# maxsonate/video-diffusion-nnx

Measured on AMD Instinct MI355X. Metric: denoised frames/sec, 16fx64x64 1000-step DDPM, higher is better.
Workload: dtype bf16; 1 GPU; config_v2_2 (north-star shape): Unet3D dim=64 C=1, 16f x 64x64, DDPM T=1000 p_sample_loop (UNet forward + p_sample per step, hipGraph replay); value = n_gpus*B*F/(T*s_per_step); batch_per_gpu=64, parallelism=dp1 (independent samples, no collective), mfma_operands=bf16, storage=weights fp32 master, activations bf16, fp32 accumulate, process_group=none (single process)

## Files before the change

### video_diffusion_nnx_amd/csrc/conv_pw.hip

```cpp
#include "vdx_common.h"
#include "vdx_internal.h"

namespace vdx {

typedef unsigned pu32x4 __attribute__((ext_vector_type(4)));

template <int ROWS, int KS = 4, bool OUT32 = false>
__global__ __launch_bounds__(512) void conv1x1_pw_kernel(const ConvArgs P, const int nct, const int groups_per_range, const int ngroups) {
    using M = Mma<MODE_BF16>;
    constexpr int TM = ROWS / 16, TN = 2;
    constexpr int KBB = KS * 64;
    extern __shared__ __attribute__((aligned(16))) char smem[];
    const int Cin = P.C0 + P.C1, nkb = Cin / (32 * KS);
    const int WRS = Cin * 2 + 16;
    char* Wl = smem;
    float* bl = reinterpret_cast<float*>(Wl + ROWS * WRS);

    const int tid = threadIdx.x, lane = tid & 63, wave = tid >> 6, lp = lane & 15, q = lane >> 4;
    const int ct = (blockIdx.x >> 3) % nct, range = ((blockIdx.x >> 3) / nct) * 8 + (blockIdx.x & 7);
    const int co0 = ct * ROWS;
    const int g0 = range * groups_per_range, g1 = min(g0 + groups_per_range, ngroups);
    if (g0 >= g1) return;

    {
        const int cpr = Cin >> 3;
        const char* wsrc = reinterpret_cast<const char*>(P.wp);
        for (int i = tid; i < ROWS * cpr; i += 512) {
            const int row = i / cpr, c = i - row * cpr;
            const int tm = row >> 4, rr = row & 15;
            const int co = co0 + (tm >> 1) * 32 + (rr >> 2) * 8 + (tm & 1) * 4 + (rr & 3);
            *reinterpret_cast<uint4*>(Wl + row * WRS + c * 16) = *reinterpret_cast<const uint4*>(wsrc + ((size_t)(P.wrow0 + co) * P.CinPad + c * 8) * 2);
        }
        for (int i = tid; i < ROWS; i += 512) bl[i] = P.bias ? P.bias[co0 + i] : 0.f;
    }
    __syncthreads();

    const __amdgpu_buffer_rsrc_t rx0 = __builtin_amdgcn_make_buffer_rsrc(const_cast<float*>(P.x0), 0, P.x0_bytes, 0x00020000);
    const __amdgpu_buffer_rsrc_t rx1 = __builtin_amdgcn_make_buffer_rsrc(const_cast<float*>(P.C1 ? P.x1 : P.x0), 0, P.C1 ? P.x1_bytes : P.x0_bytes, 0x00020000);
    const int nkb0 = P.C0 / (32 * KS);
    const unsigned rb0 = P.C0 * 2, rb1 = P.C1 * 2;

    auto load_block = [&](int g, int kb, pu32x4 (&xf)[KS][TN]) {
        const bool second = kb >= nkb0;
        const unsigned rb = second ? rb1 : rb0;
        const unsigned base = (unsigned)(g * 32 + lp) * rb + (unsigned)((second ? kb - nkb0 : kb) * KBB + q * 16);
#pragma unroll
        for (int s = 0; s < KS; ++s)
#pragma unroll
            for (int tn = 0; tn < TN; ++tn) {
                const unsigned off = base + tn * 16 * rb + s * 64;
                xf[s][tn] = second ? __builtin_amdgcn_raw_buffer_load_b128(rx1, off, 0, 0) : __builtin_amdgcn_raw_buffer_load_b128(rx0, off, 0, 0);
            }
    };
    f32x4 acc[TM][TN];
    auto mma_block = [&](int kb, const pu32x4 (&xf)[KS][TN]) {
#pragma unroll
        for (int s = 0; s < KS; ++s) {
            uint4 bf[TN];
#pragma unroll
            for (int tn = 0; tn < TN; ++tn) bf[tn] = make_uint4(xf[s][tn].x, xf[s][tn].y, xf[s][tn].z, xf[s][tn].w);
#pragma unroll
            for (int tm = 0; tm < TM; ++tm) {
                const uint4 af = *reinterpret_cast<const uint4*>(Wl + (tm * 16 + lp) * WRS + kb * KBB + s * 64 + q * 16);
#pragma unroll
                for (int tn = 0; tn < TN; ++tn) M::mma(acc[tm][tn], af, bf[tn]);
            }
        }
    };

    char* const yb = reinterpret_cast<char*>(P.y);
    const char* const resb = reinterpret_cast<const char*>(P.res);
    constexpr bool PP = ROWS == 64 && KS == 4;
    auto init_acc = [&]() {
#pragma unroll
        for (int tm = 0; tm < TM; ++tm) {
            const float4 b4 = *reinterpret_cast<const float4*>(bl + (tm >> 1) * 32 + q * 8 + (tm & 1) * 4);
#pragma unroll
            for (int tn = 0; tn < TN; ++tn) acc[tm][tn] = f32x4{b4.x, b4.y, b4.z, b4.w};
        }
    };
    auto store_group = [&](int g) {
#pragma unroll
        for (int tn = 0; tn < TN; ++tn) {
            const size_t pix = (size_t)g * 32 + tn * 16 + lp;
#pragma unroll
            for (int j = 0; j < TM / 2; ++j) {
                const size_t el = pix * P.Cout + co0 + j * 32 + q * 8;
                float o[8];
#pragma unroll
                for (int k = 0; k < 4; ++k) { o[k] = acc[2 * j][tn][k]; o[4 + k] = acc[2 * j + 1][tn][k]; }
                if constexpr (OUT32) {
                    if (resb) {
                        const float4 r0 = *reinterpret_cast<const float4*>(resb + el * 4), r1 = *reinterpret_cast<const float4*>(resb + el * 4 + 16);
                        o[0] += r0.x; o[1] += r0.y; o[2] += r0.z; o[3] += r0.w; o[4] += r1.x; o[5] += r1.y; o[6] += r1.z; o[7] += r1.w;
                    }
                    *reinterpret_cast<float4*>(yb + el * 4) = make_float4(o[0], o[1], o[2], o[3]);
                    *reinterpret_cast<float4*>(yb + el * 4 + 16) = make_float4(o[4], o[5], o[6], o[7]);
                } else {
                    const size_t e = el * 2;
                    if (resb) {
                        const uint4 r = *reinterpret_cast<const uint4*>(resb + e);
                        o[0] += __uint_as_float(r.x << 16); o[1] += __uint_as_float(r.x & 0xFFFF0000u);
                        o[2] += __uint_as_float(r.y << 16); o[3] += __uint_as_float(r.y & 0xFFFF0000u);
                        o[4] += __uint_as_float(r.z << 16); o[5] += __uint_as_float(r.z & 0xFFFF0000u);
                        o[6] += __uint_as_float(r.w << 16); o[7] += __uint_as_float(r.w & 0xFFFF0000u);
                    }
                    *reinterpret_cast<uint4*>(yb + e) = make_uint4(pack_bf16x2(o[0], o[1]), pack_bf16x2(o[2], o[3]), pack_bf16x2(o[4], o[5]), pack_bf16x2(o[6], o[7]));
                }
            }
        }
    };
    if constexpr (KS == 2) {
        pu32x4 xa[KS][TN], xb[KS][TN];
        int g = g0 + wave;
        if (g < g1) load_block(g, 0, xa);
        for (; g < g1; g += 16) {
            __asm__ volatile("" ::: "memory");
            if (g + 8 < g1) load_block(g + 8, 0, xb);
            init_acc(); mma_block(0, xa); store_group(g);
            if (g + 8 >= g1) break;
            if (g + 16 < g1) load_block(g + 16, 0, xa);
            init_acc(); mma_block(0, xb); store_group(g + 8);
        }
    } else {
        pu32x4 xa[KS][TN], xb[PP ? KS : 1][TN];
        for (int g = g0 + wave; g < g1; g += 8) {
            __asm__ volatile("" ::: "memory");
            init_acc();
            load_block(g, 0, xa);
            if constexpr (PP) {
                for (int kb = 0; kb < nkb; kb += 2) {
                    if (kb + 1 < nkb) load_block(g, kb + 1, xb);
                    mma_block(kb, xa);
                    if (kb + 1 >= nkb) break;
                    if (kb + 2 < nkb) load_block(g, kb + 2, xa);
                    mma_block(kb + 1, xb);
                }
            } else {
                for (int kb = 0; kb < nkb; ++kb) {
                    mma_block(kb, xa);
                    if (kb + 1 < nkb) load_block(g, kb + 1, xa);
                }
            }
            store_group(g);
        }
    }
}

int conv1x1_pw_rows(const ConvArgs& a) {
    const int cin = a.C0 + a.C1;
    if (a.Cout % 128 == 0 && (size_t)128 * (cin * 2 + 16) + 128 * 4 <= 140 * 1024) return 128;
    return 64;
}

bool conv1x1_pw_eligible(int mode, const ConvArgs& a) {
    if (mode != MODE_BF16 || a.kind != 0 || a.kh != 1 || a.kw != 1 || a.stride != 1 || a.pad != 0 || a.pro || a.out_stats) return false;
    if (!a.x0_bf16 || (a.C1 && !a.x1_bf16)) return false;
    const bool out32 = !a.y_bf16;
    if (a.res && (a.res_bf16 != 0) == out32) return false;
    const int cin = a.C0 + a.C1;
    if ((cin % 128 && cin != 64) || cin > 1024 || a.Cout % 64 || a.Cout < 64) return false;
    if (out32 && cin == 64) return false;
    if (!out32 && cin != 64 && a.Cout < 128) return false;
    if (a.C1 && (a.C0 % 128 || a.C1 % 128)) return false;
    if (a.CinPad != cin) return false;
    const size_t npix = (size_t)a.NF * a.H * a.W;
    if (npix % 32 || npix < 32 * 256) return false;
    if (npix * (size_t)std::max(std::max(a.C0, a.C1), a.Cout) * 2 >= 0xFFFF0000ull) return false;
    const int rows = conv1x1_pw_rows(a);
    if ((size_t)rows * (cin * 2 + 16) + rows * 4 > 160 * 1024) return false;
    return true;
}

hipError_t launch_conv1x1_pw(const ConvArgs& a, hipStream_t st) {
    const int cin = a.C0 + a.C1, rows = conv1x1_pw_rows(a), nct = a.Cout / rows;
    const int ngroups = (int)((size_t)a.NF * a.H * a.W / 32);
    const int cus = device_cus();
    const size_t lds = (size_t)rows * (cin * 2 + 16) + rows * 4;
    const int wg_per_cu = (lds <= 80 * 1024 && rows == 128) ? 2 : 1;
    int nranges = std::max(8, (cus * wg_per_cu / nct) / 8 * 8);
    int gpr = ((ngroups + nranges - 1) / nranges + 7) / 8 * 8;
    nranges = ((ngroups + gpr - 1) / gpr + 7) / 8 * 8;
    auto go = [&](auto kfn) -> hipError_t {
        if (hipError_t e = lds_opt_in(kfn, lds); e != hipSuccess) return e;
        hipLaunchKernelGGL(kfn, dim3(nranges * nct), dim3(512), lds, st, a, nct, gpr, ngroups);
        return hipGetLastError();
    };
    if (!a.y_bf16) return rows == 128 ? go(conv1x1_pw_kernel<128, 4, true>) : go(conv1x1_pw_kernel<64, 4, true>);
    if (cin == 64) return rows == 128 ? go(conv1x1_pw_kernel<128, 2>) : go(conv1x1_pw_kernel<64, 2>);
    return rows == 128 ? go(conv1x1_pw_kernel<128>) : go(conv1x1_pw_kernel<64>);
}

}
```

Before: 49.72 frames/s.

## Double-buffer pointwise conv K-loop across groups and prefetch residual early

Extends the register double-buffered K-block pipeline from only the 64-row/KS4 variant to all KS=4 variants. For most variants it also prefetches the next group's first K-block during the current group's last block, using out-of-bounds buffer offsets to keep loads branch-free. Residual loads for bf16 outputs are issued before the MMA loop so their latency is hidden, and sched_barriers pin the load/MMA interleave. This costs more VGPRs for the second buffer and residual registers, which may lower occupancy for the 128-row tiles.

```diff
diff --git a/video_diffusion_nnx_amd/csrc/conv_pw.hip b/video_diffusion_nnx_amd/csrc/conv_pw.hip
--- a/video_diffusion_nnx_amd/csrc/conv_pw.hip
+++ b/video_diffusion_nnx_amd/csrc/conv_pw.hip
@@ -9,6 +9,7 @@
 __global__ __launch_bounds__(512) void conv1x1_pw_kernel(const ConvArgs P, const int nct, const int groups_per_range, const int ngroups) {
     using M = Mma<MODE_BF16>;
     constexpr int TM = ROWS / 16, TN = 2;
+    constexpr bool XG = !(OUT32 && ROWS == 128);
     constexpr int KBB = KS * 64;
     extern __shared__ __attribute__((aligned(16))) char smem[];
     const int Cin = P.C0 + P.C1, nkb = Cin / (32 * KS);
@@ -40,17 +41,16 @@
     const int nkb0 = P.C0 / (32 * KS);
     const unsigned rb0 = P.C0 * 2, rb1 = P.C1 * 2;
 
-    auto load_block = [&](int g, int kb, pu32x4 (&xf)[KS][TN]) {
+    constexpr unsigned OOB = 0xFFFF0000u;
+    auto load_block = [&](int g, int kb, pu32x4 (&xf)[KS][TN], bool live = true) {
         const bool second = kb >= nkb0;
         const unsigned rb = second ? rb1 : rb0;
-        const unsigned base = (unsigned)(g * 32 + lp) * rb + (unsigned)((second ? kb - nkb0 : kb) * KBB + q * 16);
+        const unsigned base = live ? (unsigned)(g * 32 + lp) * rb + (unsigned)((second ? kb - nkb0 : kb) * KBB + q * 16) : OOB;
+        const __amdgpu_buffer_rsrc_t rx = second ? rx1 : rx0;
 #pragma unroll
         for (int s = 0; s < KS; ++s)
 #pragma unroll
-            for (int tn = 0; tn < TN; ++tn) {
-                const unsigned off = base + tn * 16 * rb + s * 64;
-                xf[s][tn] = second ? __builtin_amdgcn_raw_buffer_load_b128(rx1, off, 0, 0) : __builtin_amdgcn_raw_buffer_load_b128(rx0, off, 0, 0);
-            }
+            for (int tn = 0; tn < TN; ++tn) xf[s][tn] = __builtin_amdgcn_raw_buffer_load_b128(rx, base + tn * 16 * rb + s * 64, 0, 0);
     };
     f32x4 acc[TM][TN];
     auto mma_block = [&](int kb, const pu32x4 (&xf)[KS][TN]) {
@@ -70,7 +70,6 @@
 
     char* const yb = reinterpret_cast<char*>(P.y);
     const char* const resb = reinterpret_cast<const char*>(P.res);
-    constexpr bool PP = ROWS == 64 && KS == 4;
     auto init_acc = [&]() {
 #pragma unroll
         for (int tm = 0; tm < TM; ++tm) {
@@ -79,7 +78,21 @@
             for (int tn = 0; tn < TN; ++tn) acc[tm][tn] = f32x4{b4.x, b4.y, b4.z, b4.w};
         }
     };
-    auto store_group = [&](int g) {
+    constexpr int RV = OUT32 ? 2 : 1;
+    auto load_res = [&](int g, uint4 (&rr)[TN][TM / 2][RV]) {
+        if (!resb) return;
+#pragma unroll
+        for (int tn = 0; tn < TN; ++tn) {
+            const size_t pix = (size_t)g * 32 + tn * 16 + lp;
+#pragma unroll
+            for (int j = 0; j < TM / 2; ++j) {
+                const size_t e = (pix * P.Cout + co0 + j * 32 + q * 8) * (OUT32 ? 4 : 2);
+#pragma unroll
+                for (int v = 0; v < RV; ++v) rr[tn][j][v] = *reinterpret_cast<const uint4*>(resb + e + v * 16);
+            }
+        }
+    };
+    auto store_group = [&](int g, const uint4 (&rr)[TN][TM / 2][RV]) {
 #pragma unroll
         for (int tn = 0; tn < TN; ++tn) {
             const size_t pix = (size_t)g * 32 + tn * 16 + lp;
@@ -91,15 +104,16 @@
                 for (int k = 0; k < 4; ++k) { o[k] = acc[2 * j][tn][k]; o[4 + k] = acc[2 * j + 1][tn][k]; }
                 if constexpr (OUT32) {
                     if (resb) {
-                        const float4 r0 = *reinterpret_cast<const float4*>(resb + el * 4), r1 = *reinterpret_cast<const float4*>(resb + el * 4 + 16);
-                        o[0] += r0.x; o[1] += r0.y; o[2] += r0.z; o[3] += r0.w; o[4] += r1.x; o[5] += r1.y; o[6] += r1.z; o[7] += r1.w;
+                        const uint4 r0 = rr[tn][j][0], r1 = rr[tn][j][RV - 1];
+                        o[0] += __uint_as_float(r0.x); o[1] += __uint_as_float(r0.y); o[2] += __uint_as_float(r0.z); o[3] += __uint_as_float(r0.w);
+                        o[4] += __uint_as_float(r1.x); o[5] += __uint_as_float(r1.y); o[6] += __uint_as_float(r1.z); o[7] += __uint_as_float(r1.w);
                     }
                     *reinterpret_cast<float4*>(yb + el * 4) = make_float4(o[0], o[1], o[2], o[3]);
                     *reinterpret_cast<float4*>(yb + el * 4 + 16) = make_float4(o[4], o[5], o[6], o[7]);
                 } else {
                     const size_t e = el * 2;
                     if (resb) {
-                        const uint4 r = *reinterpret_cast<const uint4*>(resb + e);
+                        const uint4 r = KS == 2 ? *reinterpret_cast<const uint4*>(resb + e) : rr[tn][j][0];
                         o[0] += __uint_as_float(r.x << 16); o[1] += __uint_as_float(r.x & 0xFFFF0000u);
                         o[2] += __uint_as_float(r.y << 16); o[3] += __uint_as_float(r.y & 0xFFFF0000u);
                         o[4] += __uint_as_float(r.z << 16); o[5] += __uint_as_float(r.z & 0xFFFF0000u);
@@ -110,6 +124,7 @@
             }
         }
     };
+    uint4 rr[TN][TM / 2][RV];
     if constexpr (KS == 2) {
         pu32x4 xa[KS][TN], xb[KS][TN];
         int g = g0 + wave;
@@ -117,32 +132,34 @@
         for (; g < g1; g += 16) {
             __asm__ volatile("" ::: "memory");
             if (g + 8 < g1) load_block(g + 8, 0, xb);
-            init_acc(); mma_block(0, xa); store_group(g);
+            init_acc(); mma_block(0, xa); store_group(g, rr);
             if (g + 8 >= g1) break;
             if (g + 16 < g1) load_block(g + 16, 0, xa);
-            init_acc(); mma_block(0, xb); store_group(g + 8);
+            init_acc(); mma_block(0, xb); store_group(g + 8, rr);
         }
     } else {
-        pu32x4 xa[KS][TN], xb[PP ? KS : 1][TN];
-        for (int g = g0 + wave; g < g1; g += 8) {
+        pu32x4 xa[KS][TN], xb[KS][TN];
+        int g = g0 + wave;
+        if constexpr (XG) load_block(g, 0, xa, g < g1);
+        for (; g < g1; g += 8) {
             __asm__ volatile("" ::: "memory");
+            if constexpr (!XG) load_block(g, 0, xa);
+            if constexpr (!OUT32) load_res(g, rr);
             init_acc();
-            load_block(g, 0, xa);
-            if constexpr (PP) {
-                for (int kb = 0; kb < nkb; kb += 2) {
-                    if (kb + 1 < nkb) load_block(g, kb + 1, xb);
-                    mma_block(kb, xa);
-                    if (kb + 1 >= nkb) break;
-                    if (kb + 2 < nkb) load_block(g, kb + 2, xa);
-                    mma_block(kb + 1, xb);
-                }
-            } else {
-                for (int kb = 0; kb < nkb; ++kb) {
-                    mma_block(kb, xa);
-                    if (kb + 1 < nkb) load_block(g, kb + 1, xa);
-                }
-            }
-            store_group(g);
+            for (int kb = 0;; kb += 2) {
+                load_block(g, kb + 1, xb, kb + 1 < nkb);
+                __builtin_amdgcn_sched_barrier(0);
+                mma_block(kb, xa);
+                const bool more = kb + 2 < nkb;
+                __builtin_amdgcn_sched_barrier(0);
+                load_block(more ? g : g + 8, more ? kb + 2 : 0, xa, more || (XG && g + 8 < g1));
+                __builtin_amdgcn_sched_barrier(0);
+                if (kb + 1 >= nkb) break;
+                mma_block(kb + 1, xb);
+                if (!more) break;
+            }
+            if constexpr (OUT32) load_res(g, rr);
+            store_group(g, rr);
         }
     }
 }
```

Result: no change. 49.72 frames/s (-0.0%).
